# jalhajj/mahout

Hardware: AMD Instinct MI355X
Metric: sketch updates/sec + item-pair cosines/sec @1M items, 1/2/4/8 MI355X (higher is better)
Workload: dtype u32

## Files before the change

### mahout_amd/csrc/cms_build.hip

```cpp
#include <hip/hip_runtime.h>

#include <algorithm>
#include <cstdlib>
#include <type_traits>

#include "cms_device.h"
#include "cms_internal.h"

namespace cms {

#ifdef CMS_BUILD_CHEAPHASH
#define bucket(hp, d, kp) ((uint32_t)(((kp) >> (d)) & (hp).wmask))
#endif
#ifdef CMS_BUILD_GATHERHASH
#define bucket(hp, d, kp) \
  ((uint32_t)(((&(hp).gtab[(kp) & 0xFFFFFFu].x)[((d) >> 1) & 3] >> (((d) & 1) << 4)) & (hp).wmask))
#endif

struct HotInfo {
  int64_t row;
  int32_t nslices;
  int32_t e0;
};

// ... 408 lines not shown
      if (m >= (1ULL << 32)) atomicOr(flags, kFlagOverflow);
    } else if (tm) {
      unsigned long long old = atomicAdd((unsigned long long*)&row_mass[row], (unsigned long long)tm);
      if (old + tm >= (1ULL << 32)) atomicOr(flags, kFlagOverflow);
    }
  }
}

constexpr int kMidThreads = 256;
constexpr int64_t kMidCachedKeys = (int64_t)kMidThreads * kKeyRegs;
constexpr int64_t kStreamBigKeys = 4096;
__device__ __forceinline__ int32_t list2_at(const int32_t* list, uint32_t cap, uint32_t nfront, uint32_t i) {
  return i < nfront ? list[i] : list[cap - 1u - (i - nfront)];
}
__host__ __device__ __forceinline__ int nib_first_bits(int64_t m, int w, int bit_keys, int crumb_keys) {
  return (m <= bit_keys && (w & 127) == 0) ? 1 : (m <= crumb_keys && (w & 63) == 0) ? 2 : 4;
}
__host__ __device__ __forceinline__ bool nib_list_row(int64_t m, int w, int d, bool weighted, int frac_bits,
                                                      int bit_keys, int crumb_keys, int list_keys) {
  return m <= list_keys && !weighted && frac_bits == 0 &&
         2 + 2 * (int64_t)d * m <= ((int64_t)d * w * nib_first_bits(m, w, bit_keys, crumb_keys)) / 8;
}
__host__ __device__ __forceinline__ bool mid_list_row(int64_t m, int w, int d, bool weighted, int frac_bits,
                                                      int list_keys) {
  return m <= list_keys && !weighted && frac_bits == 0 && (int64_t)d * m <= 8192 &&
         2 + 2 * (int64_t)d * m < (int64_t)d * w / 2;
}
enum {
  kCntSlot = 0,
  kCntMid = 1 ,
  kCntStream = 3 ,
  kCntTicket = 5,
  kCntMidLists = 6,
  kCntWords = 8
};
constexpr int kClassChunk = 4096;
__global__ __launch_bounds__(256) void k_build_classes(const int64_t* lo_, const int64_t* hi_, int64_t nrows,
                                                       const int32_t* hidx, const uint64_t* bound, int32_t* slot_list,
                                                       int32_t* mid_list, int32_t* stream_list, uint32_t* cnt,
                                                       int32_t* mid_lists, int mid_lists_keys, int d, int w) {
  __shared__ int32_t s_own[kClassChunk], s_str[kClassChunk], s_lst[kClassChunk];
  __shared__ uint32_t s_n[5], s_b[5];
  const int lane = (int)__lane_id();
  const int tid = threadIdx.x;
  const uint32_t cap = (uint32_t)nrows;
  const unsigned long long below = (1ULL << lane) - 1ULL;
  for (int64_t r0 = (int64_t)blockIdx.x * kClassChunk; r0 < nrows; r0 += (int64_t)gridDim.x * kClassChunk) {
    if (tid < 5) s_n[tid] = 0;
    __syncthreads();
    for (int64_t r = r0 + tid; r < r0 + kClassChunk; r += 256) {
      bool is[5] = {false, false, false, false, false};
      if (r < nrows) {
        const int32_t sl = hidx[r];
        const int64_t m = hi_[r] - lo_[r];
        is[0] = sl >= 0;
        const bool is_mid = !is[0] && !byte_class(sl, m, bound[r]);
        const bool cached = is_mid && m <= kMidCachedKeys;
        is[4] = cached && mid_list_row(m, w, d, false, 0, mid_lists_keys);
        is[1] = cached && !is[4];
        is[2] = is_mid && m > kStreamBigKeys;
        is[3] = is_mid && !cached && !is[2];
      }
      unsigned long long mk[5];
      uint32_t b[5] = {0, 0, 0, 0, 0};
#pragma unroll
      for (int k = 0; k < 5; ++k) {
        mk[k] = __ballot(is[k]);
        if (lane == 0 && mk[k]) b[k] = atomicAdd(&s_n[k], (uint32_t)__popcll(mk[k]));
        b[k] = (uint32_t)__shfl((int)b[k], 0, 64) + (uint32_t)__popcll(mk[k] & below);
      }
      if (is[0]) s_own[b[0]] = (int32_t)r;
      if (is[1]) s_own[kClassChunk - 1 - b[1]] = (int32_t)r;
      if (is[2]) s_str[b[2]] = (int32_t)r;
      if (is[3]) s_str[kClassChunk - 1 - b[3]] = (int32_t)r;
      if (is[4]) s_lst[b[4]] = (int32_t)r;
    }
    __syncthreads();
    if (tid < 5) {
      const int ci = tid == 0 ? kCntSlot : tid == 1 ? kCntMid + 1 : tid == 4 ? kCntMidLists : kCntStream + tid - 2;
      s_b[tid] = s_n[tid] ? atomicAdd(&cnt[ci], s_n[tid]) : 0u;
    }
    __syncthreads();
    for (uint32_t i = tid; i < s_n[0]; i += 256) slot_list[s_b[0] + i] = s_own[i];
    for (uint32_t i = tid; i < s_n[1]; i += 256) mid_list[cap - 1u - (s_b[1] + i)] = s_own[kClassChunk - 1 - i];
    for (uint32_t i = tid; i < s_n[2]; i += 256) stream_list[s_b[2] + i] = s_str[i];
    for (uint32_t i = tid; i < s_n[3]; i += 256) stream_list[cap - 1u - (s_b[3] + i)] = s_str[kClassChunk - 1 - i];
    for (uint32_t i = tid; i < s_n[4]; i += 256) mid_lists[s_b[4] + i] = s_lst[i];
    __syncthreads();
  }
}

constexpr int kMidListKeys = kBuildThreads * kKeyRegs;
constexpr int kMidRowKeys = 4;
template <int SV, int D, int MT>
__device__ __forceinline__ void mid_rows(
    const int64_t* lo_, const int64_t* hi_, const Keys& keys, const float* vals, const HashParams& hp,
    const int32_t* list, const uint32_t* list_cnt, uint32_t cap, const TableView& tv, int32_t* hidx_w,
    uint32_t* cbound, uint64_t* row_mass, uint64_t* norm, uint32_t* rowmax, uint32_t* flags, int list_keys,
    int u4_keys, int u8_keys) {
  static_assert(MT == kMidThreads, "one instantiation per depth");
  constexpr int MTH = MT;
  constexpr int MKR = kKeyRegs;
  extern __shared__ __align__(16) uint32_t lds[];
  __shared__ unsigned long long s_norm[CMS_MAX_DEPTH];
  __shared__ unsigned long long s_mass;
  __shared__ uint32_t s_max, s_ovf;
  const int tid = threadIdx.x;
  const int w = (int)hp.width;
  const uint32_t nfront = list_cnt[0], count = nfront + list_cnt[1];
  for (uint32_t li = blockIdx.x; li < count; li += gridDim.x) {
    const int64_t row = list2_at(list, cap, nfront, li);
    const int64_t lo = lo_[row], hi = hi_[row];
    const bool cached = (hi - lo) <= (int64_t)MTH * MKR;
    uint64_t kp[MKR];
    uint32_t ik[MKR];
    uint64_t mass = 0;
    bool badv = false;
    if (cached) {
#pragma unroll
      for (int k = 0; k < MKR; ++k) {
// ... 248 lines not shown
      nx[u] = i < end ? load(i) : R(0);
    }
  };
  if (lo < end) fetch(lo);
  for (int64_t base = lo; base < end; base += kStep) {
    R kk[PER];
#pragma unroll
    for (int u = 0; u < PER; ++u) kk[u] = nx[u];
    if (base + kStep < end) fetch(base + kStep);
    const int live = (int)min(end - base, kStep);
    if constexpr (std::is_same<typename std::decay<G>::type, NoRedo>::value) {
#pragma unroll
      for (int u = 0; u < PER; ++u)
        if (tid < live - u * T) f(kk[u]);
    } else {
      uint32_t left = 0;
#pragma unroll
      for (int u = 0; u < PER; ++u)
        if (tid < live - u * T && f(kk[u])) left |= 1u << u;
      if (left) {
#pragma unroll 1
        for (int u = 0; u < PER; ++u) {
          if (!((left >> u) & 1u)) continue;
          R k = kk[0];
#pragma unroll
          for (int j = 1; j < PER; ++j) k = j == u ? kk[j] : k;
          g(k);
        }
      }
    }
  }
}

constexpr int kStreamThreads = 512;
constexpr int kStreamPer = 2;
constexpr int kStreamRedWords = 1 + (kStreamThreads / 64) * (CMS_MAX_DEPTH + 2);
template <int SV, int D>
__device__ __forceinline__ void mid_streamed(const int64_t* lo_, const int64_t* hi_, const Keys& keys,
                                             const HashParams& hp, const int32_t* list, const uint32_t* list_cnt,
                                             uint32_t cap, const TableView& tv, int32_t* hidx_w, uint32_t* cbound,
                                             uint64_t* row_mass, uint64_t* norm, uint32_t* rowmax, int32_t* redo,
                                             uint32_t* redo_cnt, uint32_t* ticket, int u4_keys, int u8_keys) {
  extern __shared__ __align__(16) uint32_t lds[];
  constexpr int T = kStreamThreads;
  constexpr int NW = T / 64;
  constexpr int RS = CMS_MAX_DEPTH + 2;
  const int tid = threadIdx.x, lane = tid & 63, wv = tid >> 6;
  const int w = (int)hp.width;
  const int depth = D > 0 ? D : hp.depth;
  const int nq = w >> 4;
  const uint32_t nfront = list_cnt[0], count = nfront + list_cnt[1];
  uint4* l4 = reinterpret_cast<uint4*>(lds);
  uint32_t* red = lds + 1;
  if (tid == 0) lds[0] = atomicAdd(ticket, 1u);
  __syncthreads();
  uint32_t li = lds[0];
  while (li < count) {
    __syncthreads();
    const int64_t row = list2_at(list, cap, nfront, li);
    const int64_t lo = lo_[row], hi = hi_[row];
    const int64_t m = hi - lo;
    const bool u8_start = m > u4_keys && m <= u8_keys;
    uint32_t mine = 0;
    uint32_t bytes = 0;
    u16x2 pm = {0, 0};
    if (u8_start) {
      for (int j = tid; j < depth * nq; j += T) l4[j] = make_uint4(0, 0, 0, 0);
      __syncthreads();
      auto add = [&](int r, uint32_t bk) {
        const uint32_t c = (uint32_t)r * (uint32_t)w + bk;
        atomicAdd(&lds[c >> 2], 1u << ((c & 3u) << 3));
      };
      constexpr int DR = D > 0 ? D : 1;
      const RowHash<DR> rh(hp);
      const bool fast = kRowHash && D > 0 && hp.fastq, tok = keys.tok != nullptr;
      key_pass<uint64_t, kStreamPer, T>(
          lo, hi, tid, [&](int64_t i) { return keys.raw(i); },
          [&](uint64_t raw) {
            if (!fast) {
              each_bucket<(kRowHash ? 0 : D)>(hp, keys.resolve(raw), add);
              return false;
            }
            uint32_t bk[DR];
            uint32_t k = (uint32_t)raw;
            bool again = k >= kTokEscape;
            if (!tok) {
              const uint64_t kp = reduce_key((int64_t)raw);
              k = (uint32_t)kp;
              again = kp >= kRowHashKeyEnd;
            }
            if (rh.rows32(k, bk) || again) {
              const uint64_t kp = keys.resolve(raw);
#pragma unroll 1
              for (int r = 0; r < D; ++r) add(r, bucket(hp, r, kp));
              return false;
            }
#pragma unroll
            for (int r = 0; r < D; ++r)
              atomicAdd(reinterpret_cast<uint32_t*>(reinterpret_cast<char*>(lds) + ((uint32_t)r * (uint32_t)w + (bk[r] & ~3u))),
                        1u << ((bk[r] << 3) & 31u));
            return false;
          },
          NoRedo{});
      __syncthreads();
      uint4* d4 = reinterpret_cast<uint4*>(tv.row16(row));
      auto sweep_row = [&](int r) {
        uint32_t sq = 0;
        for (int j = tid; j < nq; j += T) {
          const uint4 v = l4[r * nq + j];
          const uint32_t x[4] = {v.x, v.y, v.z, v.w};
#pragma unroll
          for (int q = 0; q < 4; ++q) {
            sq = __builtin_amdgcn_udot4(x[q], x[q], sq, false);
            bytes = __builtin_amdgcn_udot4(x[q], 0x01010101u, bytes, false);
            pm = __builtin_elementwise_max(pm, __builtin_elementwise_max(__builtin_bit_cast(u16x2, x[q] & 0x00FF00FFu),
                                                                         __builtin_bit_cast(u16x2, (x[q] >> 8) & 0x00FF00FFu)));
          }
          store_row(d4 + r * nq + j, v, SV);
        }
        sq = wave_sum_u32(sq);
        if (lane == r) mine = sq;
      };
#pragma unroll 1
      for (int r = 0; r < depth; ++r) sweep_row(r);
    }
    uint32_t vmax = max((uint32_t)pm.x, (uint32_t)pm.y);
#pragma unroll
    for (int o = 32; o > 0; o >>= 1) vmax = max(vmax, (uint32_t)__shfl_xor((int)vmax, o, 64));
    bytes = wave_sum_u32(bytes);
    __syncthreads();
    if (lane < depth) red[wv * RS + lane] = mine;
    if (lane == 0) {
      red[wv * RS + CMS_MAX_DEPTH] = vmax;
      red[wv * RS + CMS_MAX_DEPTH + 1] = bytes;
    }
    if (tid == 0) lds[0] = atomicAdd(ticket, 1u);
    __syncthreads();
    uint32_t mx = 0, total = 0;
#pragma unroll
    for (int k = 0; k < NW; ++k) {
      mx = max(mx, red[k * RS + CMS_MAX_DEPTH]);
      total += red[k * RS + CMS_MAX_DEPTH + 1];
    }
    if (!u8_start || total != (uint32_t)depth * (uint32_t)m) {
      if (tid == 0) redo[atomicAdd(redo_cnt, 1u)] = (int32_t)row;
    } else {
      if (tid < depth) {
        uint64_t s = 0;
#pragma unroll
        for (int k = 0; k < NW; ++k) s += red[k * RS + tid];
        norm[row * depth + tid] = s;
      }
      if (tid == 0) {
        rowmax[row] = mx;
        row_mass[row] = (uint64_t)m;
        hidx_w[row] = kFormU8;
        cbound[row] = mx;
      }
    }
    li = lds[0];
  }
}

template <int SV, int D, int MT>
__global__ __launch_bounds__(MT) __attribute__((amdgpu_waves_per_eu(MT == kStreamThreads ? 8 : 4, 8))) void k_build_mid(
    const int64_t* lo_, const int64_t* hi_, Keys keys, const float* vals, HashParams hp,
    const int32_t* list, const uint32_t* list_cnt , uint32_t cap, TableView tv, int32_t* hidx_w,
    uint32_t* cbound, uint64_t* row_mass, uint64_t* norm, uint32_t* rowmax, uint32_t* flags, int list_keys,
    int u4_keys, int u8_keys, int32_t* redo, uint32_t* redo_cnt, uint32_t* ticket) {
  if constexpr (MT == kStreamThreads)
    mid_streamed<SV, D>(lo_, hi_, keys, hp, list, list_cnt, cap, tv, hidx_w, cbound, row_mass, norm, rowmax, redo,
                        redo_cnt, ticket, u4_keys, u8_keys);
  else
    mid_rows<SV, D, MT>(lo_, hi_, keys, vals, hp, list, list_cnt, cap, tv, hidx_w, cbound, row_mass, norm, rowmax,
                        flags, list_keys, u4_keys, u8_keys);
}

constexpr int kMidGridPerCu = 8;
constexpr int kNibWaves = 4;

__global__ void k_row_caps(const int64_t* lo_, const int64_t* hi_, int64_t n, const uint64_t* bound,
                           const int32_t* hidx, int forms, int weighted, int frac_bits, int d, int w, int bit_keys,
                           int crumb_keys, int list_keys, uint32_t* caps) {
  const int64_t dw = (int64_t)d * w;
  const uint32_t full = (uint32_t)(slot_units(dw) / kRowAlign);
  for (int64_t r = blockIdx.x * (int64_t)blockDim.x + threadIdx.x; r < n; r += (int64_t)gridDim.x * blockDim.x) {
    const int32_t s = hidx[r];
    const int64_t m = hi_[r] - lo_[r];
    uint32_t c = full;
    if (s >= 0) {
      c = 0;
    } else if (forms && byte_class(s, m, bound[r])) {
      const int64_t u16s = nib_list_row(m, w, d, weighted != 0, frac_bits, bit_keys, crumb_keys, list_keys)
                               ? 1 + (int64_t)d * m
                               : dw / 2;
      c = (uint32_t)((u16s + kRowAlign - 1) / kRowAlign);
    }
    caps[r] = c;
  }
}

template <int SV>
__device__ __forceinline__ void nib_owner(
    int64_t row, uint32_t* lds, const int64_t* lo_, const int64_t* hi_, const Keys& keys, const float* vals,
    const HashParams& hp, const int32_t* row_hot, const uint64_t* bound, const TableView& tv, int32_t* hidx_w,
// ... 68 lines not shown
    }
    if (!__ballot(ovf) || bits == 4) break;
    bits *= 2;
  }
  if (as_list && lane == 0) lst[0] = (uint16_t)m;
  if (badv) atomicOr(flags, kFlagBadValue);
  if (__ballot(ovf)) {
    if (lane == 0) redo[atomicAdd(redo_cnt, 1u)] = as_list ? ~(int32_t)row : (int32_t)row;
    return;
  }
#pragma unroll
  for (int o = 32; o > 0; o >>= 1) vmax = max(vmax, (uint32_t)__shfl_xor((int)vmax, o, 64));
  mass = wave_sum_u32(mass);
  if (lane == 0) {
    rowmax[row] = vmax;
    row_mass[row] = mass;
    hidx_w[row] = as_list ? kFormList : bits == 1 ? kFormU1 : bits == 2 ? kFormU2 : kFormU4;
    cbound[row] = vmax;
  }
}


template <int SV, int>
__global__ __launch_bounds__(64 * kNibWaves) __attribute__((amdgpu_waves_per_eu(8, 8))) void k_build_nibbles(
    const int64_t* lo_, const int64_t* hi_, Keys keys, const float* vals, int64_t nrows, HashParams hp,
    const int32_t* row_hot, const uint64_t* bound, TableView tv, int32_t* hidx_w, uint32_t* cbound, uint64_t* row_mass,
    uint64_t* norm, uint32_t* rowmax, uint32_t* flags, int32_t* redo, uint32_t* redo_cnt, int bit_keys,
    int crumb_keys, int list_keys, int lists_done) {
  extern __shared__ __align__(16) uint32_t lds[];
  const int64_t nw = (int64_t)gridDim.x * kNibWaves;
  for (int64_t row = (int64_t)blockIdx.x * kNibWaves + (threadIdx.x >> 6); row < nrows; row += nw)
    nib_owner<SV>(row, lds, lo_, hi_, keys, vals, hp, row_hot, bound, tv, hidx_w, cbound, row_mass, norm, rowmax, flags,
                  redo, redo_cnt, bit_keys, crumb_keys, list_keys, lists_done);
}

template <typename F>
__device__ __forceinline__ uint32_t wave_fold_dpp(uint32_t v, F f) {
  v = f(v, (uint32_t)__builtin_amdgcn_update_dpp(0, (int)v, 0xB1, 0xF, 0xF, true));
  v = f(v, (uint32_t)__builtin_amdgcn_update_dpp(0, (int)v, 0x4E, 0xF, 0xF, true));
  v = f(v, (uint32_t)__builtin_amdgcn_update_dpp(0, (int)v, 0x141, 0xF, 0xF, true));
  v = f(v, (uint32_t)__builtin_amdgcn_update_dpp(0, (int)v, 0x140, 0xF, 0xF, true));
  v = f(v, (uint32_t)__builtin_amdgcn_update_dpp(0, (int)v, 0x142, 0xA, 0xF, false));
  v = f(v, (uint32_t)__builtin_amdgcn_update_dpp(0, (int)v, 0x143, 0xC, 0xF, false));
  return (uint32_t)__builtin_amdgcn_readlane((int)v, 63);
}

template <int D, int NS>
__device__ __forceinline__ bool list_rows(uint32_t* slot, const uint32_t (&pk)[kKeyRegs][(D + 1) / 2], int lane,
                                          int m, uint32_t (&sq)[3], uint32_t& vmax) {
  const uint32_t tail = lane + 64 * (NS - 1) < m ? 1u : 0u;
  bool ovf = false;
#pragma unroll
  for (int r = 0; r < D; ++r) {
    uint32_t c[NS], old[NS];
#pragma unroll
    for (int k = 0; k < NS; ++k) {
      c[k] = (pk[k][r >> 1] >> ((r & 1) << 4)) & 0xFFFFu;
      old[k] = atomicAdd(&slot[c[k] >> 3], (k < NS - 1 ? 1u : tail) << ((c[k] & 7u) << 2));
    }
#pragma unroll
    for (int k = 0; k < NS; ++k) {
      const uint32_t live = k < NS - 1 ? 1u : tail;
      const uint32_t o = (old[k] >> ((c[k] & 7u) << 2)) & 15u;
      const uint32_t nv = (o + 1u) * live;
      ovf |= nv > 15u;
      sq[r >> 1] += ((2u * o + 1u) * live) << ((r & 1) << 4);
      vmax = max(vmax, nv);
      slot[c[k] >> 3] = 0u;
    }
    if (__ballot(ovf)) return true;
  }
  return false;
}

template <int SV, int D>
__global__ __launch_bounds__(64 * kNibWaves) __attribute__((amdgpu_waves_per_eu(8, 8))) void k_build_lists(
    const int64_t* lo_, const int64_t* hi_, Keys keys, int64_t nrows, HashParams hp, const int32_t* row_hot,
// ... 681 lines not shown
  bool hot_norms_done = false;
  auto launch_hot_norms = [&]() -> int {
    TimedScope ts(h, "hot_norms");
    dim3 grid((unsigned)std::max<int64_t>(1, std::min<int64_t>(max_hot, 1024)), (unsigned)h->p.depth);
    hipLaunchKernelGGL(k_hot_norms, grid, dim3(256), 0, h->stream, hot, counters, h->hp, h->tview(), h->d_norm,
                       h->d_rowmax, whole_slices);
    CMS_HIP(hipGetLastError());
    hot_norms_done = true;
    return CMS_OK;
  };
  {
    TimedScope ts(h, "build_rows");
    auto kern = k_build_rows<kBuildStoreForm>;
    auto launch_slices = [&]() -> int {
      if (!fast_slices) return CMS_OK;
#ifdef CMS_BUILD_SKIP_SLICES
      return CMS_OK;
#endif
      static bool attr = [] {
        for (const void* f : {(const void*)k_build_slices<0>, (const void*)k_build_slices<4>,
                              (const void*)k_build_slices<5>})
          (void)hipFuncSetAttribute(f, hipFuncAttributeMaxDynamicSharedMemorySize, 80 * 1024);
        return true;
      }();
      (void)attr;
      auto kslices = h->p.depth == 5 ? k_build_slices<5> : h->p.depth == 4 ? k_build_slices<4> : k_build_slices<0>;
      hipLaunchKernelGGL(kslices, dim3((unsigned)emax), dim3(kSliceThreads), img_lds, h->stream, d_lo, d_hi,
                         keys, h->hp, kSliceKeys, hot, extra_map, counters, h->tview(), h->d_row_mass, h->d_flags,
                         whole_slices, h->d_norm, h->d_rowmax);
      CMS_HIP(hipGetLastError());
      return CMS_OK;
    };
    if (forms) {
      CMS_HIP(h->ws_blist.ensure(sizeof(int32_t) * (size_t)(4 * n + kCntWords)));
      int32_t* slot_list = h->ws_blist.as<int32_t>();
      int32_t* mid_list = slot_list + n;
      int32_t* stream_list = mid_list + n;
      int32_t* mid_lists = stream_list + n;
      uint32_t* lcnt = reinterpret_cast<uint32_t*>(mid_lists + n);
      CMS_HIP(h->ws_plist.ensure(sizeof(int32_t) * (size_t)(n + 1)));
      int32_t* redo = h->ws_plist.as<int32_t>();
      uint32_t* redo_cnt = reinterpret_cast<uint32_t*>(redo + n);
#if defined(CMS_BUILD_CHEAPHASH) || defined(CMS_BUILD_GATHERHASH)
      const int lists_done = 0;
#else
      const int lists_done = !d_val && h->hp.frac_bits == 0 && h->hp.fastq && lists_allowed(h) &&
                                     (h->p.depth == 4 || h->p.depth == 5)
                                 ? 1
                                 : 0;
#endif
      const bool mid_lists_done = lists_done && h->p.width <= kMidListSlotMax;
      CMS_HIP(hipMemsetAsync(lcnt, 0, kCntWords * sizeof(uint32_t), h->stream));
      CMS_HIP(hipMemsetAsync(redo_cnt, 0, sizeof(uint32_t), h->stream));
      hipLaunchKernelGGL(k_build_classes,
                         dim3((unsigned)std::max<int64_t>(1, std::min<int64_t>((n + kClassChunk - 1) / kClassChunk, 1024))),
                         dim3(256), 0, h->stream, d_lo, d_hi, n, h->d_hidx, h->ws_bound.as<uint64_t>(), slot_list,
                         mid_list, stream_list, lcnt, mid_lists, mid_lists_done ? kMidListKeys : 0, h->p.depth,
                         h->p.width);
      CMS_HIP(hipGetLastError());
      if (h->plan_side_active) return set_error(CMS_E_STATE, "internal: side stream used while swapped for the plan");
      hipStream_t side = h->side_stream ? h->side_stream : h->stream;
#ifdef CMS_BUILD_SERIAL
      side = h->stream;
#endif
      const hipStream_t side2 = side != h->stream && h->tune.build_streams >= 3 ? h->side_stream2 : side;
      struct SideJoin {
        cms_handle* h;
        hipStream_t side, side2;
        bool armed = false;
        ~SideJoin() {
          if (armed && hipEventRecord(h->ev_join2, side) == hipSuccess)
            (void)hipStreamWaitEvent(h->stream, h->ev_join2, 0);
          if (armed && side2 != side && hipEventRecord(h->ev_join3, side2) == hipSuccess)
            (void)hipStreamWaitEvent(h->stream, h->ev_join3, 0);
        }
      } join{h, side, side2};
      if (side != h->stream) {
        CMS_HIP(hipEventRecord(h->ev_fork2, h->stream));
        CMS_HIP(hipStreamWaitEvent(side, h->ev_fork2, 0));
        if (side2 != side) CMS_HIP(hipStreamWaitEvent(side2, h->ev_fork2, 0));
        join.armed = true;
      }
      const int64_t nib_blocks = (n + kNibWaves - 1) / kNibWaves;
      const size_t nib_lds = (size_t)kNibWaves * (size_t)h->p.width / 2;
      if (mid_lists_done) {
        auto kml = h->p.depth == 5 ? k_build_mid_lists<kBuildStoreForm, 5> : k_build_mid_lists<kBuildStoreForm, 4>;
        const size_t ml_lds = (size_t)kMidListWaves * (size_t)h->p.width;
        if (h->mid_lists_wgs_per_cu <= 0) {
          int per_cu = 0;
          CMS_HIP(hipOccupancyMaxActiveBlocksPerMultiprocessor(&per_cu, kml, 64 * kMidListWaves, ml_lds));
          h->mid_lists_wgs_per_cu = std::max(1, per_cu);
// ... 3 lines not shown
        hipLaunchKernelGGL(kml, dim3((unsigned)ml_blocks), dim3(64 * kMidListWaves), ml_lds, side, d_lo, d_hi, keys,
                           h->hp, (const int32_t*)mid_lists, (const uint32_t*)(lcnt + kCntMidLists), h->tview(),
                           h->d_hidx, h->d_cbound, h->d_row_mass, h->d_norm, h->d_rowmax, mid_list, lcnt + kCntMid);
        CMS_HIP(hipGetLastError());
        if (side2 != side) CMS_HIP(hipEventRecord(h->ev_mid_lists, side));
      }
      if (lists_done) {
        auto klists = h->p.depth == 5 ? k_build_lists<kBuildStoreForm, 5> : k_build_lists<kBuildStoreForm, 4>;
        if (h->lists_wgs_per_cu <= 0) {
          int per_cu = 0;
          CMS_HIP(hipOccupancyMaxActiveBlocksPerMultiprocessor(&per_cu, klists, 64 * kNibWaves, nib_lds));
          h->lists_wgs_per_cu = std::max(1, per_cu);
        }
        const int64_t lists_blocks = std::min<int64_t>(nib_blocks, (int64_t)h->num_cus * h->lists_wgs_per_cu);
        hipLaunchKernelGGL(klists, dim3((unsigned)lists_blocks), dim3(64 * kNibWaves), nib_lds, side, d_lo, d_hi, keys,
                           n, h->hp, row_hot, h->ws_bound.as<uint64_t>(), h->tview(), h->d_hidx, h->d_cbound,
                           h->d_row_mass, h->d_norm, h->d_rowmax, redo, redo_cnt, h->tune.bit_keys,
                           h->tune.crumb_keys, h->tune.list_keys);
      }
      bool nibbles_idle = lists_done != 0;
      for (int64_t m = 0; nibbles_idle && m < kByteKeys; ++m)
        nibbles_idle = nib_list_row(m, h->p.width, h->p.depth, false, 0, h->tune.bit_keys, h->tune.crumb_keys,
                                    h->tune.list_keys);
      if (!nibbles_idle)
        hipLaunchKernelGGL((k_build_nibbles<kBuildStoreForm, 0>), dim3((unsigned)nib_blocks), dim3(64 * kNibWaves),
                           nib_lds, side, d_lo, d_hi, keys, d_val, n, h->hp, row_hot, h->ws_bound.as<uint64_t>(),
                           h->tview(), h->d_hidx, h->d_cbound, h->d_row_mass, h->d_norm, h->d_rowmax, h->d_flags,
                           redo, redo_cnt, h->tune.bit_keys, h->tune.crumb_keys,
                           lists_allowed(h) ? h->tune.list_keys : 0, lists_done);
      const size_t mid_lds = std::max<size_t>((size_t)h->p.width * 2, (size_t)h->dw / 2);
      auto kmid = h->p.depth == 5   ? k_build_mid<kBuildStoreForm, 5, kMidThreads>
                  : h->p.depth == 4 ? k_build_mid<kBuildStoreForm, 4, kMidThreads>
                                    : k_build_mid<kBuildStoreForm, 0, kMidThreads>;
      auto launch_mid = [&](auto kern, int threads, unsigned grid, size_t klds, const int32_t* list, uint32_t* cnt) {
        hipLaunchKernelGGL(kern, dim3(grid), dim3(threads), klds, side2, d_lo, d_hi, keys, d_val, h->hp, list,
                           (const uint32_t*)cnt, (uint32_t)n, h->tview(), h->d_hidx, h->d_cbound, h->d_row_mass,
                           h->d_norm, h->d_rowmax, h->d_flags, lists_allowed(h) ? kMidListKeys : 0,
                           h->tune.mid_u4_keys, h->tune.mid_u8_keys, mid_list, lcnt + kCntMid, lcnt + kCntTicket);
      };
      const unsigned mid_grid = (unsigned)std::min<int64_t>(n, (int64_t)h->num_cus * kMidGridPerCu);
      bool one_pass = !d_val && h->hp.frac_bits == 0;
#ifdef CMS_BUILD_NO_STREAMED
      one_pass = false;
#endif
      if (one_pass) {
        auto kstr = h->p.depth == 5   ? k_build_mid<kBuildStoreForm, 5, kStreamThreads>
                    : h->p.depth == 4 ? k_build_mid<kBuildStoreForm, 4, kStreamThreads>
                                      : k_build_mid<kBuildStoreForm, 0, kStreamThreads>;
        const size_t str_lds = std::max<size_t>((size_t)h->dw, sizeof(uint32_t) * kStreamRedWords);
        if (h->stream_wgs_per_cu <= 0) {
          int per_cu = 0;
          CMS_HIP(hipOccupancyMaxActiveBlocksPerMultiprocessor(&per_cu, kstr, kStreamThreads, str_lds));
          h->stream_wgs_per_cu = std::max(1, per_cu);
        }
        launch_mid(kstr, kStreamThreads, (unsigned)std::min<int64_t>(n, (int64_t)h->num_cus * h->stream_wgs_per_cu),
                   str_lds, stream_list, lcnt + kCntStream);
      } else {
        launch_mid(kmid, kMidThreads, mid_grid, mid_lds, stream_list, lcnt + kCntStream);
      }
      if (mid_lists_done && side2 != side) CMS_HIP(hipStreamWaitEvent(side2, h->ev_mid_lists, 0));
      launch_mid(kmid, kMidThreads, mid_grid, mid_lds, mid_list, lcnt + kCntMid);
      hipLaunchKernelGGL(k_build_bytes<kBuildStoreForm>, dim3((unsigned)std::min<int64_t>(n, (int64_t)h->num_cus * 2)),
                         dim3(kBuildThreads), (size_t)h->dw, side, d_lo, d_hi, keys, d_val, h->hp, redo, redo_cnt,
                         h->tview(), h->d_hidx, h->d_cbound, h->d_row_mass, h->d_norm, h->d_rowmax, h->d_flags);
      CMS_HIP(hipGetLastError());
      if ((rc0 = launch_slices())) return rc0;
      const int64_t nslot = std::min<int64_t>(n, h->hot_used);
      hipLaunchKernelGGL(kern, dim3((unsigned)(row_emax + nslot)), dim3(kBuildThreads), lds, h->stream, d_lo, d_hi,
                         keys, d_val, n, h->hp, kSliceKeys, row_hot, hot, extra_map, counters, row_emax, h->tview(),
                         h->d_row_mass, h->d_norm, h->d_rowmax, h->d_flags, accumulate, slices_done,
                         h->ws_bound.as<uint64_t>(), forms, skip_untouched, h->d_hidx, h->d_cbound,
                         (const int32_t*)slot_list, (const uint32_t*)lcnt);
      CMS_HIP(hipGetLastError());
      if (join.armed) {
        join.armed = false;
        CMS_HIP(hipEventRecord(h->ev_join2, side));
        CMS_HIP(hipStreamWaitEvent(h->stream, h->ev_join2, 0));
        if (side2 != side) {
          CMS_HIP(hipEventRecord(h->ev_join3, side2));
          CMS_HIP(hipStreamWaitEvent(h->stream, h->ev_join3, 0));
        }
      }
    } else {
      if ((rc0 = launch_slices())) return rc0;
      hipLaunchKernelGGL(kern, dim3((unsigned)(row_emax + n)), dim3(kBuildThreads), lds, h->stream, d_lo, d_hi, keys,
                         d_val, n, h->hp, kSliceKeys, row_hot, hot, extra_map, counters, row_emax, h->tview(),
                         h->d_row_mass, h->d_norm, h->d_rowmax, h->d_flags, accumulate, slices_done,
                         h->ws_bound.as<uint64_t>(), forms, skip_untouched, h->d_hidx, h->d_cbound,
                         (const int32_t*)nullptr, (const uint32_t*)nullptr);
// ... 11 lines not shown
```

### mahout_amd/csrc/cms_internal.h

```cpp
#pragma once
#include <hip/hip_runtime.h>
#include <rccl/rccl.h>

#include <functional>
#include <map>
#include <mutex>
#include <shared_mutex>
#include <string>
#include <vector>

#include "../../include/mahout_cms.h"
#include "cms_forms.h"
#include "cms_hash.h"

namespace cms {

enum : uint32_t {
  kFlagBadRow = 1u << 0,
  kFlagBadValue = 1u << 1,
  kFlagOverflow = 1u << 2,
};

struct DevBuf {
  void* ptr = nullptr;
// ... 124 lines not shown
};
}

namespace cms {
struct Tunables {
  int bit_keys = 64;
  int crumb_keys = 256;
  int list_keys = 256;
  int mid_u4_keys = 768;
  int mid_u8_keys = 12288;
  int plan_side = 1;
  int build_streams = 3;
  int po_dense_x4 = 4;
  int po_bound_part2 = 1;
  int po_bound_rows = 1;
  int po_no_prune = 0;
  int po_no_bigq = 0;
  int split_keys = 0;
  bool forms = true;
  bool no_compact = false;
  bool no_vmm = false;
  bool hot_routing = true;
  bool fp4 = true;
  bool mls = true;
  int64_t threshold_slab_rows = 0;
};
}

struct cms_handle {
  cms_params p{};
  cms::Tunables tune;
  int device = 0;
  int num_cus = 256;
  int stream_wgs_per_cu = 0;
  int lists_wgs_per_cu = 0;
  int mid_lists_wgs_per_cu = 0;
  hipStream_t stream = nullptr;
  hipStream_t side_stream = nullptr;
  hipEvent_t ev_fork2 = nullptr, ev_join2 = nullptr;
  hipStream_t side_stream2 = nullptr;
  hipEvent_t ev_join3 = nullptr;
  hipEvent_t ev_mid_lists = nullptr;
  hipEvent_t ev_spans = nullptr, ev_plan = nullptr;
  bool spans_event = false, plan_side_request = false;
  bool plan_side_active = false;
  std::shared_mutex mu;
  std::mutex pool_mu;
  std::vector<cms::QueryCtx*> qpool;

  int64_t a[CMS_MAX_DEPTH] = {};
  int64_t b[CMS_MAX_DEPTH] = {};
  cms::HashParams hp{};

  int64_t n = 0;
  int64_t dw = 0;
  uint16_t* d_t16 = nullptr;
  int64_t t16_cap = 0, t16_used = 0;
  int64_t* d_off = nullptr;
  struct ArenaChunk {
    hipMemGenericAllocationHandle_t mem;
    size_t bytes;
  };
  void* arena_va = nullptr;
  size_t arena_va_bytes = 0, arena_mapped = 0, arena_gran = 0;
  int arena_small_layouts = 0;
  std::vector<ArenaChunk> arena_chunks;
  bool compact = false;
// ... 366 lines not shown
```

Baseline: 63.35 billion.

## Add u16 LDS-image streamed build path for large mid rows with token route

Rows above the u8 key limit are classified into a new u16 list and built in one pass with a 16-bit counter image in LDS, instead of being sent to the redo path. Rows whose u8 image overflows go to a carry list. The u8 streamed kernel also fetches the next row's ticket and bounds ahead of time, gets a specialised token-key hashing route, and uses DPP wave reductions. This is meant to cut redo and fallback work and the per-row latency stalls, at the cost of more LDS per workgroup (up to 80KB for the u16 image), lower occupancy for that kernel, and more kernel instantiations.

```diff
diff --git a/mahout_amd/csrc/cms_build.hip b/mahout_amd/csrc/cms_build.hip
--- a/mahout_amd/csrc/cms_build.hip
+++ b/mahout_amd/csrc/cms_build.hip
@@ -464,24 +464,27 @@
   kCntStream = 3 ,
   kCntTicket = 5,
   kCntMidLists = 6,
-  kCntWords = 8
+  kCntU16 = 7,
+  kCntTicket16 = 8,
+  kCntWords = 10
 };
 constexpr int kClassChunk = 4096;
 __global__ __launch_bounds__(256) void k_build_classes(const int64_t* lo_, const int64_t* hi_, int64_t nrows,
                                                        const int32_t* hidx, const uint64_t* bound, int32_t* slot_list,
                                                        int32_t* mid_list, int32_t* stream_list, uint32_t* cnt,
-                                                       int32_t* mid_lists, int mid_lists_keys, int d, int w) {
+                                                       int32_t* mid_lists, int mid_lists_keys, int d, int w,
+                                                       int32_t* u16_list, int64_t u16_from) {
   __shared__ int32_t s_own[kClassChunk], s_str[kClassChunk], s_lst[kClassChunk];
-  __shared__ uint32_t s_n[5], s_b[5];
+  __shared__ uint32_t s_n[6], s_b[6];
   const int lane = (int)__lane_id();
   const int tid = threadIdx.x;
   const uint32_t cap = (uint32_t)nrows;
   const unsigned long long below = (1ULL << lane) - 1ULL;
   for (int64_t r0 = (int64_t)blockIdx.x * kClassChunk; r0 < nrows; r0 += (int64_t)gridDim.x * kClassChunk) {
-    if (tid < 5) s_n[tid] = 0;
+    if (tid < 6) s_n[tid] = 0;
     __syncthreads();
     for (int64_t r = r0 + tid; r < r0 + kClassChunk; r += 256) {
-      bool is[5] = {false, false, false, false, false};
+      bool is[6] = {false, false, false, false, false, false};
       if (r < nrows) {
         const int32_t sl = hidx[r];
         const int64_t m = hi_[r] - lo_[r];
@@ -490,13 +493,14 @@
         const bool cached = is_mid && m <= kMidCachedKeys;
         is[4] = cached && mid_list_row(m, w, d, false, 0, mid_lists_keys);
         is[1] = cached && !is[4];
-        is[2] = is_mid && m > kStreamBigKeys;
-        is[3] = is_mid && !cached && !is[2];
-      }
-      unsigned long long mk[5];
-      uint32_t b[5] = {0, 0, 0, 0, 0};
-#pragma unroll
-      for (int k = 0; k < 5; ++k) {
+        is[5] = is_mid && !cached && m > u16_from;
+        is[2] = is_mid && !is[5] && m > kStreamBigKeys;
+        is[3] = is_mid && !cached && !is[5] && !is[2];
+      }
+      unsigned long long mk[6];
+      uint32_t b[6] = {0, 0, 0, 0, 0, 0};
+#pragma unroll
+      for (int k = 0; k < 6; ++k) {
         mk[k] = __ballot(is[k]);
         if (lane == 0 && mk[k]) b[k] = atomicAdd(&s_n[k], (uint32_t)__popcll(mk[k]));
         b[k] = (uint32_t)__shfl((int)b[k], 0, 64) + (uint32_t)__popcll(mk[k] & below);
@@ -506,10 +510,15 @@
       if (is[2]) s_str[b[2]] = (int32_t)r;
       if (is[3]) s_str[kClassChunk - 1 - b[3]] = (int32_t)r;
       if (is[4]) s_lst[b[4]] = (int32_t)r;
+      if (is[5]) s_lst[kClassChunk - 1 - b[5]] = (int32_t)r;
     }
     __syncthreads();
-    if (tid < 5) {
-      const int ci = tid == 0 ? kCntSlot : tid == 1 ? kCntMid + 1 : tid == 4 ? kCntMidLists : kCntStream + tid - 2;
+    if (tid < 6) {
+      const int ci = tid == 0   ? kCntSlot
+                     : tid == 1 ? kCntMid + 1
+                     : tid == 4 ? kCntMidLists
+                     : tid == 5 ? kCntU16
+                                : kCntStream + tid - 2;
       s_b[tid] = s_n[tid] ? atomicAdd(&cnt[ci], s_n[tid]) : 0u;
     }
     __syncthreads();
@@ -518,6 +527,7 @@
     for (uint32_t i = tid; i < s_n[2]; i += 256) stream_list[s_b[2] + i] = s_str[i];
     for (uint32_t i = tid; i < s_n[3]; i += 256) stream_list[cap - 1u - (s_b[3] + i)] = s_str[kClassChunk - 1 - i];
     for (uint32_t i = tid; i < s_n[4]; i += 256) mid_lists[s_b[4] + i] = s_lst[i];
+    for (uint32_t i = tid; i < s_n[5]; i += 256) u16_list[s_b[5] + i] = s_lst[kClassChunk - 1 - i];
     __syncthreads();
   }
 }
@@ -832,78 +842,170 @@
   }
 }
 
+template <typename F>
+__device__ __forceinline__ uint32_t wave_fold_dpp(uint32_t v, F f) {
+  v = f(v, (uint32_t)__builtin_amdgcn_update_dpp(0, (int)v, 0xB1, 0xF, 0xF, true));
+  v = f(v, (uint32_t)__builtin_amdgcn_update_dpp(0, (int)v, 0x4E, 0xF, 0xF, true));
+  v = f(v, (uint32_t)__builtin_amdgcn_update_dpp(0, (int)v, 0x141, 0xF, 0xF, true));
+  v = f(v, (uint32_t)__builtin_amdgcn_update_dpp(0, (int)v, 0x140, 0xF, 0xF, true));
+  v = f(v, (uint32_t)__builtin_amdgcn_update_dpp(0, (int)v, 0x142, 0xA, 0xF, false));
+  v = f(v, (uint32_t)__builtin_amdgcn_update_dpp(0, (int)v, 0x143, 0xC, 0xF, false));
+  return (uint32_t)__builtin_amdgcn_readlane((int)v, 63);
+}
+
 constexpr int kStreamThreads = 512;
 constexpr int kStreamPer = 2;
-constexpr int kStreamRedWords = 1 + (kStreamThreads / 64) * (CMS_MAX_DEPTH + 2);
-template <int SV, int D>
+constexpr int kStreamTokPer8 = 2, kStreamTokPer16 = 8, kStreamPer16 = 4;
+constexpr int kStreamRedWords = 1 + (kStreamThreads / 64) * (CMS_MAX_DEPTH + 2) + 5;
+constexpr size_t kStreamLds16Max = 80 * 1024;
+template <int SV, int D, int CB, bool TOK>
 __device__ __forceinline__ void mid_streamed(const int64_t* lo_, const int64_t* hi_, const Keys& keys,
                                              const HashParams& hp, const int32_t* list, const uint32_t* list_cnt,
                                              uint32_t cap, const TableView& tv, int32_t* hidx_w, uint32_t* cbound,
                                              uint64_t* row_mass, uint64_t* norm, uint32_t* rowmax, int32_t* redo,
-                                             uint32_t* redo_cnt, uint32_t* ticket, int u4_keys, int u8_keys) {
+                                             uint32_t* redo_cnt, int32_t* carry, uint32_t* carry_cnt, uint32_t* ticket,
+                                             int u4_keys, int u8_keys) {
+  static_assert(CB == 1 || CB == 2, "a u8 or a u16 image");
+  static_assert(!TOK || D == 4 || D == 5, "the token route is RowHash's");
   extern __shared__ __align__(16) uint32_t lds[];
   constexpr int T = kStreamThreads;
   constexpr int NW = T / 64;
   constexpr int RS = CMS_MAX_DEPTH + 2;
+  constexpr int DR = D > 0 ? D : 1;
   const int tid = threadIdx.x, lane = tid & 63, wv = tid >> 6;
   const int w = (int)hp.width;
   const int depth = D > 0 ? D : hp.depth;
-  const int nq = w >> 4;
-  const uint32_t nfront = list_cnt[0], count = nfront + list_cnt[1];
+  const int nq = (w * CB) >> 4;
+  const uint32_t nfront = list_cnt[0], count = nfront + (CB == 1 ? list_cnt[1] : 0u);
   uint4* l4 = reinterpret_cast<uint4*>(lds);
   uint32_t* red = lds + 1;
-  if (tid == 0) lds[0] = atomicAdd(ticket, 1u);
+  auto add = [&](int r, uint32_t bk) {
+    const uint32_t c = (uint32_t)r * (uint32_t)w + bk;
+    if constexpr (CB == 1) atomicAdd(&lds[c >> 2], 1u << ((c & 3u) << 3));
+    else atomicAdd(&lds[c >> 1], 1u << ((c & 1u) << 4));
+  };
+  auto add_rows = [&](const uint32_t (&bk)[DR]) {
+#pragma unroll
+    for (int r = 0; r < DR; ++r) {
+      if constexpr (CB == 1)
+        atomicAdd(reinterpret_cast<uint32_t*>(reinterpret_cast<char*>(lds) + ((uint32_t)r * (uint32_t)w + (bk[r] & ~3u))),
+                  1u << ((bk[r] << 3) & 31u));
+      else
+        atomicAdd(reinterpret_cast<uint32_t*>(reinterpret_cast<char*>(lds) +
+                                              ((uint32_t)r * (2u * (uint32_t)w) | ((bk[r] << 1) & ~3u))),
+                  1u << ((bk[r] << 4) & 31u));
+    }
+  };
+  RowHash<DR> rhv(hp);
+  if constexpr (TOK) rhv.vgpr();
+  constexpr bool AHEAD = CB == 1;
+  uint32_t* nxt = red + NW * RS;
+  uint32_t t2 = 0, t3 = 0;
+  auto publish = [&](uint32_t t, int32_t row, int64_t lo, int64_t hi) {
+    lds[0] = t;
+    nxt[0] = (uint32_t)row;
+    nxt[1] = (uint32_t)lo;
+    nxt[2] = (uint32_t)((uint64_t)lo >> 32);
+    nxt[3] = (uint32_t)hi;
+    nxt[4] = (uint32_t)((uint64_t)hi >> 32);
+  };
+  if (tid == 0) {
+    const uint32_t t = atomicAdd(ticket, 1u);
+    if constexpr (AHEAD) {
+      const int32_t r0 = t < count ? list2_at(list, cap, nfront, t) : 0;
+      publish(t, r0, t < count ? lo_[r0] : 0, t < count ? hi_[r0] : 0);
+      t2 = atomicAdd(ticket, 1u);
+    } else {
+      lds[0] = t;
+    }
+  }
   __syncthreads();
   uint32_t li = lds[0];
   while (li < count) {
+    int64_t row, lo, hi;
+    if constexpr (AHEAD) {
+      row = __builtin_amdgcn_readfirstlane((int)nxt[0]);
+      lo = (int64_t)((uint64_t)(uint32_t)__builtin_amdgcn_readfirstlane((int)nxt[1]) |
+                     (uint64_t)(uint32_t)__builtin_amdgcn_readfirstlane((int)nxt[2]) << 32);
+      hi = (int64_t)((uint64_t)(uint32_t)__builtin_amdgcn_readfirstlane((int)nxt[3]) |
+                     (uint64_t)(uint32_t)__builtin_amdgcn_readfirstlane((int)nxt[4]) << 32);
+    }
     __syncthreads();
-    const int64_t row = list2_at(list, cap, nfront, li);
-    const int64_t lo = lo_[row], hi = hi_[row];
+    if constexpr (!AHEAD) {
+      row = list2_at(list, cap, nfront, li);
+      lo = lo_[row];
+      hi = hi_[row];
+    }
+    int32_t nrow = 0;
+    if constexpr (AHEAD) {
+      if (tid == 0) {
+        if (t2 < count) nrow = list2_at(list, cap, nfront, t2);
+        t3 = atomicAdd(ticket, 1u);
+      }
+    }
+    uint4* d4 = reinterpret_cast<uint4*>(tv.row16(row));
     const int64_t m = hi - lo;
-    const bool u8_start = m > u4_keys && m <= u8_keys;
+    const bool build = CB == 2 || (m > u4_keys && m <= u8_keys);
     uint32_t mine = 0;
     uint32_t bytes = 0;
     u16x2 pm = {0, 0};
-    if (u8_start) {
+    if (build) {
       for (int j = tid; j < depth * nq; j += T) l4[j] = make_uint4(0, 0, 0, 0);
       __syncthreads();
-      auto add = [&](int r, uint32_t bk) {
-        const uint32_t c = (uint32_t)r * (uint32_t)w + bk;
-        atomicAdd(&lds[c >> 2], 1u << ((c & 3u) << 3));
-      };
-      constexpr int DR = D > 0 ? D : 1;
-      const RowHash<DR> rh(hp);
-      const bool fast = kRowHash && D > 0 && hp.fastq, tok = keys.tok != nullptr;
-      key_pass<uint64_t, kStreamPer, T>(
-          lo, hi, tid, [&](int64_t i) { return keys.raw(i); },
-          [&](uint64_t raw) {
-            if (!fast) {
-              each_bucket<(kRowHash ? 0 : D)>(hp, keys.resolve(raw), add);
+      if constexpr (TOK) {
+        const uint32_t* tok = keys.tok;
+        key_pass<uint32_t, (CB == 1 ? kStreamTokPer8 : kStreamTokPer16), T>(
+            lo, hi, tid, [&](int64_t i) { return tok[i]; },
+            [&](uint32_t t) {
+              uint32_t bk[DR];
+              if (rhv.rows32(t, bk) || t >= kTokEscape) return true;
+              add_rows(bk);
               return false;
-            }
-            uint32_t bk[DR];
-            uint32_t k = (uint32_t)raw;
-            bool again = k >= kTokEscape;
-            if (!tok) {
-              const uint64_t kp = reduce_key((int64_t)raw);
-              k = (uint32_t)kp;
-              again = kp >= kRowHashKeyEnd;
-            }
-            if (rh.rows32(k, bk) || again) {
-              const uint64_t kp = keys.resolve(raw);
+            },
+            [&](uint32_t t) {
+              const uint64_t kp = keys.resolve(t);
 #pragma unroll 1
               for (int r = 0; r < D; ++r) add(r, bucket(hp, r, kp));
+            });
+      } else {
+        const RowHash<DR> rh(hp);
+        const bool fast = kRowHash && D > 0 && hp.fastq, tok = keys.tok != nullptr;
+        key_pass<uint64_t, (CB == 1 ? kStreamPer : kStreamPer16), T>(
+            lo, hi, tid, [&](int64_t i) { return keys.raw(i); },
+            [&](uint64_t raw) {
+              if (!fast) {
+                each_bucket<(kRowHash ? 0 : D)>(hp, keys.resolve(raw), add);
+                return false;
+              }
+              uint32_t bk[DR];
+              uint32_t k = (uint32_t)raw;
+              bool again = k >= kTokEscape;
+              if (!tok) {
+                const uint64_t kp = reduce_key((int64_t)raw);
+                k = (uint32_t)kp;
+                again = kp >= kRowHashKeyEnd;
+              }
+              if (rh.rows32(k, bk) || again) {
+                const uint64_t kp = keys.resolve(raw);
+#pragma unroll 1
+                for (int r = 0; r < D; ++r) add(r, bucket(hp, r, kp));
+                return false;
+              }
+              add_rows(bk);
               return false;
-            }
-#pragma unroll
-            for (int r = 0; r < D; ++r)
-              atomicAdd(reinterpret_cast<uint32_t*>(reinterpret_cast<char*>(lds) + ((uint32_t)r * (uint32_t)w + (bk[r] & ~3u))),
-                        1u << ((bk[r] << 3) & 31u));
-            return false;
-          },
-          NoRedo{});
+            },
+            NoRedo{});
+      }
       __syncthreads();
-      uint4* d4 = reinterpret_cast<uint4*>(tv.row16(row));
+    }
+    int64_t nlo = 0, nhi = 0;
+    if constexpr (AHEAD) {
+      if (tid == 0 && t2 < count) {
+        nlo = lo_[nrow];
+        nhi = hi_[nrow];
+      }
+    }
+    if (build) {
       auto sweep_row = [&](int r) {
         uint32_t sq = 0;
         for (int j = tid; j < nq; j += T) {
@@ -911,30 +1013,41 @@
           const uint32_t x[4] = {v.x, v.y, v.z, v.w};
 #pragma unroll
           for (int q = 0; q < 4; ++q) {
-            sq = __builtin_amdgcn_udot4(x[q], x[q], sq, false);
-            bytes = __builtin_amdgcn_udot4(x[q], 0x01010101u, bytes, false);
-            pm = __builtin_elementwise_max(pm, __builtin_elementwise_max(__builtin_bit_cast(u16x2, x[q] & 0x00FF00FFu),
-                                                                         __builtin_bit_cast(u16x2, (x[q] >> 8) & 0x00FF00FFu)));
+            if constexpr (CB == 1) {
+              sq = __builtin_amdgcn_udot4(x[q], x[q], sq, false);
+              bytes = __builtin_amdgcn_udot4(x[q], 0x01010101u, bytes, false);
+              pm = __builtin_elementwise_max(pm, __builtin_elementwise_max(__builtin_bit_cast(u16x2, x[q] & 0x00FF00FFu),
+                                                                           __builtin_bit_cast(u16x2, (x[q] >> 8) & 0x00FF00FFu)));
+            } else {
+              const u16x2 c = __builtin_bit_cast(u16x2, x[q]);
+              sq = __builtin_amdgcn_udot2(c, c, sq, false);
+              pm = __builtin_elementwise_max(pm, c);
+            }
           }
           store_row(d4 + r * nq + j, v, SV);
         }
-        sq = wave_sum_u32(sq);
+        sq = wave_fold_dpp(sq, [](uint32_t a, uint32_t b) { return a + b; });
         if (lane == r) mine = sq;
       };
 #pragma unroll 1
       for (int r = 0; r < depth; ++r) sweep_row(r);
     }
-    uint32_t vmax = max((uint32_t)pm.x, (uint32_t)pm.y);
-#pragma unroll
-    for (int o = 32; o > 0; o >>= 1) vmax = max(vmax, (uint32_t)__shfl_xor((int)vmax, o, 64));
-    bytes = wave_sum_u32(bytes);
+    const uint32_t vmax = wave_fold_dpp(max((uint32_t)pm.x, (uint32_t)pm.y), [](uint32_t a, uint32_t b) { return max(a, b); });
+    bytes = wave_fold_dpp(bytes, [](uint32_t a, uint32_t b) { return a + b; });
     __syncthreads();
     if (lane < depth) red[wv * RS + lane] = mine;
     if (lane == 0) {
       red[wv * RS + CMS_MAX_DEPTH] = vmax;
       red[wv * RS + CMS_MAX_DEPTH + 1] = bytes;
     }
-    if (tid == 0) lds[0] = atomicAdd(ticket, 1u);
+    if (tid == 0) {
+      if constexpr (AHEAD) {
+        publish(t2, nrow, nlo, nhi);
+        t2 = t3;
+      } else {
+        lds[0] = atomicAdd(ticket, 1u);
+      }
+    }
     __syncthreads();
     uint32_t mx = 0, total = 0;
 #pragma unroll
@@ -942,8 +1055,10 @@
       mx = max(mx, red[k * RS + CMS_MAX_DEPTH]);
       total += red[k * RS + CMS_MAX_DEPTH + 1];
     }
-    if (!u8_start || total != (uint32_t)depth * (uint32_t)m) {
+    if (!build) {
       if (tid == 0) redo[atomicAdd(redo_cnt, 1u)] = (int32_t)row;
+    } else if (CB == 1 && total != (uint32_t)depth * (uint32_t)m) {
+      if (tid == 0) carry[atomicAdd(carry_cnt, 1u)] = (int32_t)row;
     } else {
       if (tid < depth) {
         uint64_t s = 0;
@@ -954,7 +1069,7 @@
       if (tid == 0) {
         rowmax[row] = mx;
         row_mass[row] = (uint64_t)m;
-        hidx_w[row] = kFormU8;
+        hidx_w[row] = CB == 1 ? kFormU8 : kFormU16;
         cbound[row] = mx;
       }
     }
@@ -962,15 +1077,17 @@
   }
 }
 
-template <int SV, int D, int MT>
-__global__ __launch_bounds__(MT) __attribute__((amdgpu_waves_per_eu(MT == kStreamThreads ? 8 : 4, 8))) void k_build_mid(
+constexpr int mid_waves(int mt, int cb, bool tok) { return mt != kStreamThreads || cb == 2 ? 4 : tok ? 6 : 8; }
+template <int SV, int D, int MT, int CB = 0, bool TOK = false>
+__global__ __launch_bounds__(MT) __attribute__((amdgpu_waves_per_eu(mid_waves(MT, CB, TOK), 8))) void k_build_mid(
     const int64_t* lo_, const int64_t* hi_, Keys keys, const float* vals, HashParams hp,
     const int32_t* list, const uint32_t* list_cnt , uint32_t cap, TableView tv, int32_t* hidx_w,
     uint32_t* cbound, uint64_t* row_mass, uint64_t* norm, uint32_t* rowmax, uint32_t* flags, int list_keys,
-    int u4_keys, int u8_keys, int32_t* redo, uint32_t* redo_cnt, uint32_t* ticket) {
+    int u4_keys, int u8_keys, int32_t* redo, uint32_t* redo_cnt, int32_t* carry, uint32_t* carry_cnt,
+    uint32_t* ticket) {
   if constexpr (MT == kStreamThreads)
-    mid_streamed<SV, D>(lo_, hi_, keys, hp, list, list_cnt, cap, tv, hidx_w, cbound, row_mass, norm, rowmax, redo,
-                        redo_cnt, ticket, u4_keys, u8_keys);
+    mid_streamed<SV, D, CB, TOK>(lo_, hi_, keys, hp, list, list_cnt, cap, tv, hidx_w, cbound, row_mass, norm, rowmax,
+                                 redo, redo_cnt, carry, carry_cnt, ticket, u4_keys, u8_keys);
   else
     mid_rows<SV, D, MT>(lo_, hi_, keys, vals, hp, list, list_cnt, cap, tv, hidx_w, cbound, row_mass, norm, rowmax,
                         flags, list_keys, u4_keys, u8_keys);
@@ -1105,17 +1222,6 @@
   for (int64_t row = (int64_t)blockIdx.x * kNibWaves + (threadIdx.x >> 6); row < nrows; row += nw)
     nib_owner<SV>(row, lds, lo_, hi_, keys, vals, hp, row_hot, bound, tv, hidx_w, cbound, row_mass, norm, rowmax, flags,
                   redo, redo_cnt, bit_keys, crumb_keys, list_keys, lists_done);
-}
-
-template <typename F>
-__device__ __forceinline__ uint32_t wave_fold_dpp(uint32_t v, F f) {
-  v = f(v, (uint32_t)__builtin_amdgcn_update_dpp(0, (int)v, 0xB1, 0xF, 0xF, true));
-  v = f(v, (uint32_t)__builtin_amdgcn_update_dpp(0, (int)v, 0x4E, 0xF, 0xF, true));
-  v = f(v, (uint32_t)__builtin_amdgcn_update_dpp(0, (int)v, 0x141, 0xF, 0xF, true));
-  v = f(v, (uint32_t)__builtin_amdgcn_update_dpp(0, (int)v, 0x140, 0xF, 0xF, true));
-  v = f(v, (uint32_t)__builtin_amdgcn_update_dpp(0, (int)v, 0x142, 0xA, 0xF, false));
-  v = f(v, (uint32_t)__builtin_amdgcn_update_dpp(0, (int)v, 0x143, 0xC, 0xF, false));
-  return (uint32_t)__builtin_amdgcn_readlane((int)v, 63);
 }
 
 template <int D, int NS>
@@ -1863,12 +1969,19 @@
       return CMS_OK;
     };
     if (forms) {
-      CMS_HIP(h->ws_blist.ensure(sizeof(int32_t) * (size_t)(4 * n + kCntWords)));
+      CMS_HIP(h->ws_blist.ensure(sizeof(int32_t) * (size_t)(5 * n + kCntWords)));
       int32_t* slot_list = h->ws_blist.as<int32_t>();
       int32_t* mid_list = slot_list + n;
       int32_t* stream_list = mid_list + n;
       int32_t* mid_lists = stream_list + n;
-      uint32_t* lcnt = reinterpret_cast<uint32_t*>(mid_lists + n);
+      int32_t* u16_list = mid_lists + n;
+      uint32_t* lcnt = reinterpret_cast<uint32_t*>(u16_list + n);
+      bool one_pass = !d_val && h->hp.frac_bits == 0;
+#ifdef CMS_BUILD_NO_STREAMED
+      one_pass = false;
+#endif
+      const bool image16 = one_pass && (size_t)h->dw * 2 <= kStreamLds16Max;
+      const int64_t u16_from = image16 ? std::max(h->tune.mid_u8_keys, h->tune.mid_u4_keys) : INT64_MAX;
       CMS_HIP(h->ws_plist.ensure(sizeof(int32_t) * (size_t)(n + 1)));
       int32_t* redo = h->ws_plist.as<int32_t>();
       uint32_t* redo_cnt = reinterpret_cast<uint32_t*>(redo + n);
@@ -1887,7 +2000,7 @@
                          dim3((unsigned)std::max<int64_t>(1, std::min<int64_t>((n + kClassChunk - 1) / kClassChunk, 1024))),
                          dim3(256), 0, h->stream, d_lo, d_hi, n, h->d_hidx, h->ws_bound.as<uint64_t>(), slot_list,
                          mid_list, stream_list, lcnt, mid_lists, mid_lists_done ? kMidListKeys : 0, h->p.depth,
-                         h->p.width);
+                         h->p.width, u16_list, u16_from);
       CMS_HIP(hipGetLastError());
       if (h->plan_side_active) return set_error(CMS_E_STATE, "internal: side stream used while swapped for the plan");
       hipStream_t side = h->side_stream ? h->side_stream : h->stream;
@@ -1957,29 +2070,60 @@
       auto kmid = h->p.depth == 5   ? k_build_mid<kBuildStoreForm, 5, kMidThreads>
                   : h->p.depth == 4 ? k_build_mid<kBuildStoreForm, 4, kMidThreads>
                                     : k_build_mid<kBuildStoreForm, 0, kMidThreads>;
+      uint32_t* ticket = lcnt + kCntTicket;
       auto launch_mid = [&](auto kern, int threads, unsigned grid, size_t klds, const int32_t* list, uint32_t* cnt) {
         hipLaunchKernelGGL(kern, dim3(grid), dim3(threads), klds, side2, d_lo, d_hi, keys, d_val, h->hp, list,
                            (const uint32_t*)cnt, (uint32_t)n, h->tview(), h->d_hidx, h->d_cbound, h->d_row_mass,
                            h->d_norm, h->d_rowmax, h->d_flags, lists_allowed(h) ? kMidListKeys : 0,
-                           h->tune.mid_u4_keys, h->tune.mid_u8_keys, mid_list, lcnt + kCntMid, lcnt + kCntTicket);
+                           h->tune.mid_u4_keys, h->tune.mid_u8_keys, mid_list, lcnt + kCntMid,
+                           image16 ? u16_list : mid_list, image16 ? lcnt + kCntU16 : lcnt + kCntMid, ticket);
       };
       const unsigned mid_grid = (unsigned)std::min<int64_t>(n, (int64_t)h->num_cus * kMidGridPerCu);
-      bool one_pass = !d_val && h->hp.frac_bits == 0;
-#ifdef CMS_BUILD_NO_STREAMED
-      one_pass = false;
-#endif
       if (one_pass) {
-        auto kstr = h->p.depth == 5   ? k_build_mid<kBuildStoreForm, 5, kStreamThreads>
-                    : h->p.depth == 4 ? k_build_mid<kBuildStoreForm, 4, kStreamThreads>
-                                      : k_build_mid<kBuildStoreForm, 0, kStreamThreads>;
-        const size_t str_lds = std::max<size_t>((size_t)h->dw, sizeof(uint32_t) * kStreamRedWords);
-        if (h->stream_wgs_per_cu <= 0) {
-          int per_cu = 0;
-          CMS_HIP(hipOccupancyMaxActiveBlocksPerMultiprocessor(&per_cu, kstr, kStreamThreads, str_lds));
-          h->stream_wgs_per_cu = std::max(1, per_cu);
-        }
-        launch_mid(kstr, kStreamThreads, (unsigned)std::min<int64_t>(n, (int64_t)h->num_cus * h->stream_wgs_per_cu),
-                   str_lds, stream_list, lcnt + kCntStream);
+        constexpr int SV = kBuildStoreForm, T = kStreamThreads;
+        const int dep = h->p.depth;
+        const bool tok = keys.tok && kRowHash && h->hp.fastq && (dep == 4 || dep == 5);
+        auto kstr8 = tok ? (dep == 5 ? k_build_mid<SV, 5, T, 1, true> : k_build_mid<SV, 4, T, 1, true>)
+                     : dep == 5 ? k_build_mid<SV, 5, T, 1, false>
+                     : dep == 4 ? k_build_mid<SV, 4, T, 1, false>
+                                : k_build_mid<SV, 0, T, 1, false>;
+        auto kstr16 = tok ? (dep == 5 ? k_build_mid<SV, 5, T, 2, true> : k_build_mid<SV, 4, T, 2, true>)
+                      : dep == 5 ? k_build_mid<SV, 5, T, 2, false>
+                      : dep == 4 ? k_build_mid<SV, 4, T, 2, false>
+                                 : k_build_mid<SV, 0, T, 2, false>;
+        auto resident = [&](auto kern, size_t klds, int& per_cu) -> hipError_t {
+          if (per_cu <= 0) {
+            int q = 0;
+            const hipError_t e = hipOccupancyMaxActiveBlocksPerMultiprocessor(&q, kern, T, klds);
+            if (e != hipSuccess) return e;
+            per_cu = std::max(1, q);
+          }
+          return hipSuccess;
+        };
+        const size_t red_lds = sizeof(uint32_t) * kStreamRedWords;
+        const size_t lds8 = std::max<size_t>((size_t)h->dw, red_lds);
+        int& per_cu8 = h->stream_wgs_per_cu[tok ? 1 : 0];
+        CMS_HIP(resident(kstr8, lds8, per_cu8));
+        ticket = lcnt + kCntTicket;
+        launch_mid(kstr8, T, (unsigned)std::min<int64_t>(n, (int64_t)h->num_cus * per_cu8), lds8, stream_list,
+                   lcnt + kCntStream);
+        if (image16) {
+          static bool attr = [] {
+            for (const void* f : {(const void*)k_build_mid<SV, 5, T, 2, true>, (const void*)k_build_mid<SV, 4, T, 2, true>,
+                                  (const void*)k_build_mid<SV, 5, T, 2, false>, (const void*)k_build_mid<SV, 4, T, 2, false>,
+                                  (const void*)k_build_mid<SV, 0, T, 2, false>})
+              (void)hipFuncSetAttribute(f, hipFuncAttributeMaxDynamicSharedMemorySize, (int)kStreamLds16Max);
+            return true;
+          }();
+          (void)attr;
+          const size_t lds16 = std::max<size_t>((size_t)h->dw * 2, red_lds);
+          int& per_cu16 = h->stream_wgs_per_cu[tok ? 3 : 2];
+          CMS_HIP(resident(kstr16, lds16, per_cu16));
+          ticket = lcnt + kCntTicket16;
+          launch_mid(kstr16, T, (unsigned)std::min<int64_t>(n, (int64_t)h->num_cus * per_cu16), lds16, u16_list,
+                     lcnt + kCntU16);
+        }
+        ticket = lcnt + kCntTicket;
       } else {
         launch_mid(kmid, kMidThreads, mid_grid, mid_lds, stream_list, lcnt + kCntStream);
       }
diff --git a/mahout_amd/csrc/cms_internal.h b/mahout_amd/csrc/cms_internal.h
--- a/mahout_amd/csrc/cms_internal.h
+++ b/mahout_amd/csrc/cms_internal.h
@@ -180,7 +180,7 @@
   cms::Tunables tune;
   int device = 0;
   int num_cus = 256;
-  int stream_wgs_per_cu = 0;
+  int stream_wgs_per_cu[4] = {0, 0, 0, 0};
   int lists_wgs_per_cu = 0;
   int mid_lists_wgs_per_cu = 0;
   hipStream_t stream = nullptr;
```

Measured after the change: 60.63 billion. -4.3%, worse.
